# leonardsiegert/PULPo

Measured on AMD Instinct MI355X. Metric: volume-pairs/sec fwd+bwd, 160^3 fp32, higher is better.
Workload: dtype f32

## Files before the change

pulpo_amd/csrc/warp.hip:

```cpp
#include "common.h"
#include "sampling.h"

namespace {

using pulpo::Corner;
using pulpo::sample_coord;

template <int C>
__global__ __launch_bounds__(256) void warp_fwd_kernel(const float* __restrict__ df, const float* __restrict__ img, const float* __restrict__ add,
                                                         float* __restrict__ out, int B, int Dg, int Hg, int Wg, int Di, int Hi, int Wi, int Cr) {
    const long Vg = (long)Dg * Hg * Wg, Vi = (long)Di * Hi * Wi;
    const long total = (long)B * Vg;
    const int nch = C > 0 ? C : Cr;
    for (long e = blockIdx.x * (long)blockDim.x + threadIdx.x; e < total; e += (long)gridDim.x * blockDim.x) {
        const long b = B == 1 ? 0 : e / Vg, v = e - b * Vg;
        const int vi = (int)v;
        const int x = vi % Wg, y = (vi / Wg) % Hg, z = vi / (Wg * Hg);
        const float* d = df + b * 3 * Vg + v;
        const Corner cz = sample_coord((float)z, d[0], Dg, Di);
        const Corner cy = sample_coord((float)y, d[Vg], Hg, Hi);
        const Corner cx = sample_coord((float)x, d[2 * Vg], Wg, Wi);
        const long o00 = ((long)cz.i0 * Hi + cy.i0) * Wi, o01 = ((long)cz.i0 * Hi + cy.i1) * Wi;
        const long o10 = ((long)cz.i1 * Hi + cy.i0) * Wi, o11 = ((long)cz.i1 * Hi + cy.i1) * Wi;
        const float wz0 = 1.f - cz.f, wy0 = 1.f - cy.f, wx0 = 1.f - cx.f;
        for (int c = 0; c < nch; ++c) {
            const float* s = img + (b * nch + c) * Vi;
            float val = wz0 * wy0 * wx0 * s[o00 + cx.i0] + wz0 * wy0 * cx.f * s[o00 + cx.i1] + wz0 * cy.f * wx0 * s[o01 + cx.i0] +
                        wz0 * cy.f * cx.f * s[o01 + cx.i1] + cz.f * wy0 * wx0 * s[o10 + cx.i0] + cz.f * wy0 * cx.f * s[o10 + cx.i1] +
                        cz.f * cy.f * wx0 * s[o11 + cx.i0] + cz.f * cy.f * cx.f * s[o11 + cx.i1];
            const long oi = (b * nch + c) * Vg + v;
            if (add != nullptr) val += add[oi];
            out[oi] = val;
        }
    }
}

template <bool GDF_ATOMIC>
__global__ __launch_bounds__(256) void warp_bwd_kernel(const float* __restrict__ df, const float* __restrict__ img, const float* __restrict__ gout,
                                                         float* __restrict__ gdf, float* __restrict__ gimg, int B, int Dg, int Hg, int Wg, int Di,
                                                         int Hi, int Wi, int nch) {
    const long Vg = (long)Dg * Hg * Wg, Vi = (long)Di * Hi * Wi;
    const long total = (long)B * Vg;
    for (long e = blockIdx.x * (long)blockDim.x + threadIdx.x; e < total; e += (long)gridDim.x * blockDim.x) {
        const long b = B == 1 ? 0 : e / Vg, v = e - b * Vg;
        const int vi = (int)v;
        const int x = vi % Wg, y = (vi / Wg) % Hg, z = vi / (Wg * Hg);
        const float* d = df + b * 3 * Vg + v;
        const Corner cz = sample_coord((float)z, d[0], Dg, Di);
        const Corner cy = sample_coord((float)y, d[Vg], Hg, Hi);
        const Corner cx = sample_coord((float)x, d[2 * Vg], Wg, Wi);
        const long o00 = ((long)cz.i0 * Hi + cy.i0) * Wi, o01 = ((long)cz.i0 * Hi + cy.i1) * Wi;
        const long o10 = ((long)cz.i1 * Hi + cy.i0) * Wi, o11 = ((long)cz.i1 * Hi + cy.i1) * Wi;
        const float wz0 = 1.f - cz.f, wy0 = 1.f - cy.f, wx0 = 1.f - cx.f;
        float gz = 0.f, gy = 0.f, gx = 0.f;
        for (int c = 0; c < nch; ++c) {
            const float g = gout[(b * nch + c) * Vg + v];
            const float* s = img + (b * nch + c) * Vi;
            const float s000 = s[o00 + cx.i0], s001 = s[o00 + cx.i1], s010 = s[o01 + cx.i0], s011 = s[o01 + cx.i1];
            const float s100 = s[o10 + cx.i0], s101 = s[o10 + cx.i1], s110 = s[o11 + cx.i0], s111 = s[o11 + cx.i1];
            gz += g * (wy0 * wx0 * (s100 - s000) + wy0 * cx.f * (s101 - s001) + cy.f * wx0 * (s110 - s010) + cy.f * cx.f * (s111 - s011));
            gy += g * (wz0 * wx0 * (s010 - s000) + wz0 * cx.f * (s011 - s001) + cz.f * wx0 * (s110 - s100) + cz.f * cx.f * (s111 - s101));
            gx += g * (wz0 * wy0 * (s001 - s000) + wz0 * cy.f * (s011 - s010) + cz.f * wy0 * (s101 - s100) + cz.f * cy.f * (s111 - s110));
            if (gimg != nullptr) {
                float* q = gimg + (b * nch + c) * Vi;
                atomicAdd(q + o00 + cx.i0, g * wz0 * wy0 * wx0);
                atomicAdd(q + o00 + cx.i1, g * wz0 * wy0 * cx.f);
                atomicAdd(q + o01 + cx.i0, g * wz0 * cy.f * wx0);
                atomicAdd(q + o01 + cx.i1, g * wz0 * cy.f * cx.f);
                atomicAdd(q + o10 + cx.i0, g * cz.f * wy0 * wx0);
                atomicAdd(q + o10 + cx.i1, g * cz.f * wy0 * cx.f);
                atomicAdd(q + o11 + cx.i0, g * cz.f * cy.f * wx0);
                atomicAdd(q + o11 + cx.i1, g * cz.f * cy.f * cx.f);
            }
        }
        if (gdf != nullptr) {
            float* q = gdf + b * 3 * Vg + v;
            if constexpr (GDF_ATOMIC) {
                atomicAdd(q, gz * cz.dscale);
                atomicAdd(q + Vg, gy * cy.dscale);
                atomicAdd(q + 2 * Vg, gx * cx.dscale);
            } else {
                q[0] = gz * cz.dscale;
                q[Vg] = gy * cy.dscale;
                q[2 * Vg] = gx * cx.dscale;
            }
        }
    }
}

template <int R>
__global__ __launch_bounds__(256) void vecint_bwd_tile_kernel(const float* __restrict__ cur, const float* __restrict__ gout, float* __restrict__ gp,
                                                                int B, int D, int H, int W, int ntz, int nty, int ntx) {
    constexpr int TZ_ = 4, TY_ = 8, TX_ = 8;
    constexpr int BZ = TZ_ + 2 * R, BY = TY_ + 2 * R, BX = TX_ + 2 * R, BV = BZ * BY * BX;
    __shared__ float box[3 * BV];
    const int tid = threadIdx.x;
    int t = blockIdx.x;
    const int tx_ = t % ntx; t /= ntx;
    const int ty_ = t % nty; t /= nty;
    const int tz_ = t % ntz;
    const int b = t / ntz;
    const int z0 = tz_ * TZ_, y0 = ty_ * TY_, x0 = tx_ * TX_;
    const long V = (long)D * H * W;
    for (int j = tid; j < 3 * BV; j += 256) box[j] = 0.f;
    __syncthreads();
    const int z = z0 + (tid >> 6), y = y0 + ((tid >> 3) & 7), x = x0 + (tid & 7);
    const bool valid = z < D && y < H && x < W;
    const long v = valid ? ((long)z * H + y) * W + x : 0;
    const float* d = cur + (long)b * 3 * V + v;
    const Corner cz = sample_coord((float)z, valid ? d[0] : 0.f, D, D);
    const Corner cy = sample_coord((float)y, valid ? d[V] : 0.f, H, H);
    const Corner cx = sample_coord((float)x, valid ? d[2 * V] : 0.f, W, W);
    const float wz0 = 1.f - cz.f, wy0 = 1.f - cy.f, wx0 = 1.f - cx.f;
    const long o00 = ((long)cz.i0 * H + cy.i0) * W, o01 = ((long)cz.i0 * H + cy.i1) * W;
    const long o10 = ((long)cz.i1 * H + cy.i0) * W, o11 = ((long)cz.i1 * H + cy.i1) * W;
    const int lz0 = cz.i0 - z0 + R, lz1 = cz.i1 - z0 + R, ly0 = cy.i0 - y0 + R, ly1 = cy.i1 - y0 + R, lx0 = cx.i0 - x0 + R, lx1 = cx.i1 - x0 + R;
    const bool inbox = valid && lz0 >= 0 && lz1 < BZ && ly0 >= 0 && ly1 < BY && lx0 >= 0 && lx1 < BX;
    const int key = inbox ? (((lz0 * 32 + lz1) * 32 + ly0) * 32 + ly1) : -1;
    const int key_l = __shfl_up(key, 1, 64), lx1_l = __shfl_up(lx1, 1, 64);
    const bool take = inbox && (tid & 7) != 0 && key_l == key && lx1_l == lx0;
    const int take_r = __shfl_down((int)take, 1, 64);
    const bool give = (tid & 7) != 7 && take_r != 0;
    const int row = (tid >> 3) & 7;
    const int ky0 = inbox ? ((lz0 * 32 + lz1) * 32 + lx0) : -1, ky1 = (inbox && !give) ? ((lz0 * 32 + lz1) * 32 + lx1) : -1;
    const int ky0_u = __shfl_up(ky0, 8, 64), ky1_u = __shfl_up(ky1, 8, 64), ly1_u = __shfl_up(ly1, 8, 64);
    const bool take_y0 = row != 0 && ky0 >= 0 && ky0_u == ky0 && ly1_u == ly0;
    const bool take_y1 = row != 0 && ky1 >= 0 && ky1_u == ky1 && ly1_u == ly0;
    const int ty0_d = __shfl_down((int)take_y0, 8, 64), ty1_d = __shfl_down((int)take_y1, 8, 64);
    const bool give_y0 = row != 7 && ty0_d != 0, give_y1 = row != 7 && ty1_d != 0;
    float gz = 0.f, gy = 0.f, gx = 0.f;
    float gid[3];
#pragma unroll
    for (int c = 0; c < 3; ++c) {
        const float g = valid ? gout[((long)b * 3 + c) * V + v] : 0.f;
        gid[c] = g;
        if (valid) {
            const float* s = cur + ((long)b * 3 + c) * V;
            const float s000 = s[o00 + cx.i0], s001 = s[o00 + cx.i1], s010 = s[o01 + cx.i0], s011 = s[o01 + cx.i1];
            const float s100 = s[o10 + cx.i0], s101 = s[o10 + cx.i1], s110 = s[o11 + cx.i0], s111 = s[o11 + cx.i1];
            gz += g * (wy0 * wx0 * (s100 - s000) + wy0 * cx.f * (s101 - s001) + cy.f * wx0 * (s110 - s010) + cy.f * cx.f * (s111 - s011));
            gy += g * (wz0 * wx0 * (s010 - s000) + wz0 * cx.f * (s011 - s001) + cz.f * wx0 * (s110 - s100) + cz.f * cx.f * (s111 - s101));
            gx += g * (wz0 * wy0 * (s001 - s000) + wz0 * cy.f * (s011 - s010) + cz.f * wy0 * (s101 - s100) + cz.f * cy.f * (s111 - s110));
        }
        float a000 = g * wz0 * wy0 * wx0, a010 = g * wz0 * cy.f * wx0, a100 = g * cz.f * wy0 * wx0, a110 = g * cz.f * cy.f * wx0;
        const float a001 = g * wz0 * wy0 * cx.f, a011 = g * wz0 * cy.f * cx.f, a101 = g * cz.f * wy0 * cx.f, a111 = g * cz.f * cy.f * cx.f;
        const float t00 = __shfl_up(a001, 1, 64), t01 = __shfl_up(a011, 1, 64), t10 = __shfl_up(a101, 1, 64), t11 = __shfl_up(a111, 1, 64);
        if (take) { a000 += t00; a010 += t01; a100 += t10; a110 += t11; }
        float b001 = a001, b101 = a101;
        const float u010 = __shfl_up(a010, 8, 64), u110 = __shfl_up(a110, 8, 64), u011 = __shfl_up(a011, 8, 64), u111 = __shfl_up(a111, 8, 64);
        if (take_y0) { a000 += u010; a100 += u110; }
        if (take_y1) { b001 += u011; b101 += u111; }
        if (inbox) {
            float* q = box + c * BV;
            const int p00 = (lz0 * BY + ly0) * BX, p01 = (lz0 * BY + ly1) * BX, p10 = (lz1 * BY + ly0) * BX, p11 = (lz1 * BY + ly1) * BX;
            atomicAdd(q + p00 + lx0, a000);
            atomicAdd(q + p10 + lx0, a100);
            if (!give_y0) {
                atomicAdd(q + p01 + lx0, a010);
                atomicAdd(q + p11 + lx0, a110);
            }
            if (!give) {
                atomicAdd(q + p00 + lx1, b001);
                atomicAdd(q + p10 + lx1, b101);
                if (!give_y1) {
                    atomicAdd(q + p01 + lx1, a011);
                    atomicAdd(q + p11 + lx1, a111);
                }
            }
        } else if (valid) {
            float* q = gp + ((long)b * 3 + c) * V;
            atomicAdd(q + o00 + cx.i0, a000);
            atomicAdd(q + o00 + cx.i1, a001);
            atomicAdd(q + o01 + cx.i0, a010);
            atomicAdd(q + o01 + cx.i1, a011);
            atomicAdd(q + o10 + cx.i0, a100);
            atomicAdd(q + o10 + cx.i1, a101);
            atomicAdd(q + o11 + cx.i0, a110);
            atomicAdd(q + o11 + cx.i1, a111);
        }
    }
    if (valid) {
        const int own = ((z - z0 + R) * BY + (y - y0 + R)) * BX + (x - x0 + R);
        atomicAdd(box + own, gid[0] + gz * cz.dscale);
        atomicAdd(box + BV + own, gid[1] + gy * cy.dscale);
        atomicAdd(box + 2 * BV + own, gid[2] + gx * cx.dscale);
    }
    __syncthreads();
    for (int j = tid; j < 3 * BV; j += 256) {
        const float val = box[j];
        if (val == 0.f) continue;
        const int c = j / BV, r = j - c * BV;
        const int gz_ = z0 - R + r / (BY * BX), gy_ = y0 - R + (r / BX) % BY, gx_ = x0 - R + r % BX;
        if (gz_ >= 0 && gz_ < D && gy_ >= 0 && gy_ < H && gx_ >= 0 && gx_ < W)
            atomicAdd(gp + ((long)b * 3 + c) * V + ((long)gz_ * H + gy_) * W + gx_, val);
    }
}

__global__ __launch_bounds__(256) void scale_kernel(const float* __restrict__ in, float* __restrict__ out, float s, long n) {
    for (long e = blockIdx.x * (long)blockDim.x + threadIdx.x; e < n; e += (long)gridDim.x * blockDim.x) out[e] = in[e] * s;
}

constexpr int VI_THREADS = 1024, VI_MAXV = 8 * VI_THREADS;
__global__ __launch_bounds__(VI_THREADS) void vecint_fwd_lds_kernel(const float* __restrict__ v, float* __restrict__ work, int B, int D, int H, int W,
                                                                      int nsteps, float scale) {
    extern __shared__ float fld[];
    const int V = D * H * W, tid = threadIdx.x;
    const long b = blockIdx.x, n = (long)B * 3 * V;
    for (int i = tid; i < 3 * V; i += VI_THREADS) {
        const float val = v[b * 3 * V + i] * scale;
        fld[i] = val;
        work[b * 3 * V + i] = val;
    }
    __syncthreads();
    for (int k = 0; k < nsteps; ++k) {
        float nv[8][3];
#pragma unroll
        for (int j = 0; j < 8; ++j) {
            const int vox = tid + j * VI_THREADS;
            if (vox < V) pulpo::vecint_step_voxel(fld, V, vox, D, H, W, nv[j]);
        }
        __syncthreads();
        float* out = work + (long)(k + 1) * n + b * 3 * V;
#pragma unroll
        for (int j = 0; j < 8; ++j) {
            const int vox = tid + j * VI_THREADS;
            if (vox < V) {
#pragma unroll
                for (int c = 0; c < 3; ++c) {
                    fld[c * V + vox] = nv[j][c];
                    out[c * V + vox] = nv[j][c];
                }
            }
        }
        __syncthreads();
    }
}

inline int eblocks(long items) { return (int)std::max<long>(1, std::min<long>((items + 255) / 256, 8192)); }

__device__ __forceinline__ double fx_unit(const unsigned* maxbits) {
    const float m = __uint_as_float(*maxbits);
    if (!(m > 0.f) || !(m < INFINITY)) return 1.0;
    int ex;
    frexpf(m, &ex);
    return ldexp(1.0, 46 - ex);
}
__device__ __forceinline__ void fx_add(long long* p, float v, double unit) {
    atomicAdd(reinterpret_cast<unsigned long long*>(p), (unsigned long long)__double2ll_rn((double)v * unit));
}

__device__ __forceinline__ void block_absmax_to(float m, unsigned* out) {
    __shared__ float wm[4];
#pragma unroll
    for (int o = 32; o > 0; o >>= 1) m = fmaxf(m, __shfl_xor(m, o, 64));
    if ((threadIdx.x & 63) == 0) wm[threadIdx.x >> 6] = m;
    __syncthreads();
    if (threadIdx.x == 0) {
        const float t = fmaxf(fmaxf(wm[0], wm[1]), fmaxf(wm[2], wm[3]));
        if (t > 0.f) atomicMax(out, __float_as_uint(t));
    }
}
inline int fx_blocks(long items) { return (int)std::max<long>(1, std::min<long>((items + 255) / 256, 1024)); }

__global__ __launch_bounds__(256) void absmax_kernel(const float* __restrict__ g, long n, unsigned* __restrict__ out) {
    float m = 0.f;
    for (long e = blockIdx.x * (long)blockDim.x + threadIdx.x; e < n; e += (long)gridDim.x * blockDim.x) m = fmaxf(m, fabsf(g[e]));
    block_absmax_to(m, out);
}

template <bool SELF>
__global__ __launch_bounds__(256) void warp_bwd_fx_kernel(const float* __restrict__ df, const float* __restrict__ img, const float* __restrict__ gout,
                                                            float* __restrict__ gdf, long long* __restrict__ acc, const unsigned* __restrict__ maxbits,
                                                            int B, int Dg, int Hg, int Wg, int Di, int Hi, int Wi, int nch) {
    const long Vg = (long)Dg * Hg * Wg, Vi = (long)Di * Hi * Wi;
    const long total = (long)B * Vg;
    const double unit = fx_unit(maxbits);
    for (long e = blockIdx.x * (long)blockDim.x + threadIdx.x; e < total; e += (long)gridDim.x * blockDim.x) {
        const long b = B == 1 ? 0 : e / Vg, v = e - b * Vg;
        const int vi = (int)v;
        const int x = vi % Wg, y = (vi / Wg) % Hg, z = vi / (Wg * Hg);
        const float* d = df + b * 3 * Vg + v;
        const Corner cz = sample_coord((float)z, d[0], Dg, Di);
        const Corner cy = sample_coord((float)y, d[Vg], Hg, Hi);
        const Corner cx = sample_coord((float)x, d[2 * Vg], Wg, Wi);
        const long o00 = ((long)cz.i0 * Hi + cy.i0) * Wi, o01 = ((long)cz.i0 * Hi + cy.i1) * Wi;
        const long o10 = ((long)cz.i1 * Hi + cy.i0) * Wi, o11 = ((long)cz.i1 * Hi + cy.i1) * Wi;
        const float wz0 = 1.f - cz.f, wy0 = 1.f - cy.f, wx0 = 1.f - cx.f;
        float gz = 0.f, gy = 0.f, gx = 0.f;
        float gid[3] = {0.f, 0.f, 0.f};
        for (int c = 0; c < nch; ++c) {
            const float g = gout[(b * nch + c) * Vg + v];
            if (SELF && c < 3) gid[c] = g;
            const float* s = img + (b * nch + c) * Vi;
            const float s000 = s[o00 + cx.i0], s001 = s[o00 + cx.i1], s010 = s[o01 + cx.i0], s011 = s[o01 + cx.i1];
            const float s100 = s[o10 + cx.i0], s101 = s[o10 + cx.i1], s110 = s[o11 + cx.i0], s111 = s[o11 + cx.i1];
            gz += g * (wy0 * wx0 * (s100 - s000) + wy0 * cx.f * (s101 - s001) + cy.f * wx0 * (s110 - s010) + cy.f * cx.f * (s111 - s011));
            gy += g * (wz0 * wx0 * (s010 - s000) + wz0 * cx.f * (s011 - s001) + cz.f * wx0 * (s110 - s100) + cz.f * cx.f * (s111 - s101));
            gx += g * (wz0 * wy0 * (s001 - s000) + wz0 * cy.f * (s011 - s010) + cz.f * wy0 * (s101 - s100) + cz.f * cy.f * (s111 - s110));
            if (acc != nullptr) {
                long long* q = acc + (b * nch + c) * Vi;
                fx_add(q + o00 + cx.i0, g * wz0 * wy0 * wx0, unit);
                fx_add(q + o00 + cx.i1, g * wz0 * wy0 * cx.f, unit);
                fx_add(q + o01 + cx.i0, g * wz0 * cy.f * wx0, unit);
                fx_add(q + o01 + cx.i1, g * wz0 * cy.f * cx.f, unit);
                fx_add(q + o10 + cx.i0, g * cz.f * wy0 * wx0, unit);
                fx_add(q + o10 + cx.i1, g * cz.f * wy0 * cx.f, unit);
                fx_add(q + o11 + cx.i0, g * cz.f * cy.f * wx0, unit);
                fx_add(q + o11 + cx.i1, g * cz.f * cy.f * cx.f, unit);
            }
        }
        if (SELF) {
            long long* q = acc + b * 3 * Vg + v;
            fx_add(q, gid[0] + gz * cz.dscale, unit);
            fx_add(q + Vg, gid[1] + gy * cy.dscale, unit);
            fx_add(q + 2 * Vg, gid[2] + gx * cx.dscale, unit);
        } else if (gdf != nullptr) {
            float* q = gdf + b * 3 * Vg + v;
            q[0] = gz * cz.dscale;
            q[Vg] = gy * cy.dscale;
            q[2 * Vg] = gx * cx.dscale;
        }
    }
}

__global__ __launch_bounds__(256) void fx_to_float_kernel(long long* __restrict__ acc, float* __restrict__ out, long n, const unsigned* __restrict__ maxbits,
                                                            float post, unsigned* __restrict__ next_max) {
    const double inv = 1.0 / fx_unit(maxbits);
    float m = 0.f;
    for (long e = blockIdx.x * (long)blockDim.x + threadIdx.x; e < n; e += (long)gridDim.x * blockDim.x) {
        const float val = (float)((double)acc[e] * inv) * post;
        acc[e] = 0;
        out[e] = val;
        m = fmaxf(m, fabsf(val));
    }
    if (next_max != nullptr) block_absmax_to(m, next_max);
}

}

PULPO_API int pulpo_warp3d_fwd(const float* df, const float* img, float* out, int B, int C, int Dg, int Hg, int Wg, int Di, int Hi, int Wi,
                               void* stream) {
    PULPO_REQUIRE(df && img && out && B > 0 && C > 0, "warp3d_fwd: bad arguments");
    PULPO_REQUIRE(Dg >= 1 && Hg > 1 && Wg > 1 && Di > 0 && Hi > 0 && Wi > 0 && (Dg > 1 || Di == 1), "warp3d_fwd: grid H, W must be > 1 (depth 1 = 2-D form, with a depth-1 image)");
    PULPO_REQUIRE((long)Dg * Hg * Wg < (1L << 31), "warp3d_fwd: grids of 2^31 voxels and more are not supported");
    const long total = (long)B * Dg * Hg * Wg;
    hipStream_t st = (hipStream_t)stream;
    if (C == 1) hipLaunchKernelGGL(warp_fwd_kernel<1>, dim3(eblocks(total)), dim3(256), 0, st, df, img, nullptr, out, B, Dg, Hg, Wg, Di, Hi, Wi, C);
    else if (C == 3) hipLaunchKernelGGL(warp_fwd_kernel<3>, dim3(eblocks(total)), dim3(256), 0, st, df, img, nullptr, out, B, Dg, Hg, Wg, Di, Hi, Wi, C);
    else hipLaunchKernelGGL(warp_fwd_kernel<0>, dim3(eblocks(total)), dim3(256), 0, st, df, img, nullptr, out, B, Dg, Hg, Wg, Di, Hi, Wi, C);
    return pulpo::check_launch("warp3d_fwd");
}

PULPO_API int pulpo_warp3d_bwd(const float* df, const float* img, const float* gout, float* gdf, float* gimg, int B, int C, int Dg, int Hg, int Wg,
                               int Di, int Hi, int Wi, void* stream) {
    PULPO_REQUIRE(df && img && gout && B > 0 && C > 0, "warp3d_bwd: bad arguments");
    PULPO_REQUIRE(Dg >= 1 && Hg > 1 && Wg > 1 && (long)Dg * Hg * Wg < (1L << 31), "warp3d_bwd: grid H, W must be > 1 (and fewer than 2^31 voxels)");
    hipStream_t st = (hipStream_t)stream;
    if (gimg != nullptr) {
        hipError_t e = hipMemsetAsync(gimg, 0, sizeof(float) * (size_t)B * C * Di * Hi * Wi, st);
        if (e != hipSuccess) return pulpo::fail((int)e, "warp3d_bwd memset: %s", hipGetErrorString(e));
    }
    const long total = (long)B * Dg * Hg * Wg;
    hipLaunchKernelGGL(warp_bwd_kernel<false>, dim3(eblocks(total)), dim3(256), 0, st, df, img, gout, gdf, gimg, B, Dg, Hg, Wg, Di, Hi, Wi, C);
    return pulpo::check_launch("warp3d_bwd");
}

PULPO_API int pulpo_vecint_fwd(const float* v, float* work, int B, int D, int H, int W, int nsteps, void* stream) {
    PULPO_REQUIRE(v && work && B > 0 && D >= 1 && H > 1 && W > 1 && nsteps >= 0 && (long)D * H * W < (1L << 31), "vecint_fwd: bad arguments");
    hipStream_t st = (hipStream_t)stream;
    const long n = (long)B * 3 * D * H * W, total = (long)B * D * H * W;
    constexpr long VECINT_LDS_MAXV = 2048;
    static_assert(VECINT_LDS_MAXV <= VI_MAXV, "the one-launch form holds the whole field in LDS");
    if (total / B <= VECINT_LDS_MAXV && nsteps > 0) {
        const size_t lds = sizeof(float) * 3 * (size_t)(total / B);
        static bool attr_set = false;
        if (!attr_set) {
            hipError_t e = hipFuncSetAttribute(reinterpret_cast<const void*>(&vecint_fwd_lds_kernel), hipFuncAttributeMaxDynamicSharedMemorySize,
                                               (int)(sizeof(float) * 3 * VI_MAXV));
            if (e != hipSuccess) return pulpo::fail((int)e, "hipFuncSetAttribute(vecint_fwd_lds): %s", hipGetErrorString(e));
            attr_set = true;
        }
        hipLaunchKernelGGL(vecint_fwd_lds_kernel, dim3(B), dim3(VI_THREADS), lds, st, v, work, B, D, H, W, nsteps, 1.0f / (float)(1 << nsteps));
        return pulpo::check_launch("vecint_fwd_lds");
    }
    hipLaunchKernelGGL(scale_kernel, dim3(eblocks(n)), dim3(256), 0, st, v, work, 1.0f / (float)(1 << nsteps), n);
    int rc = pulpo::check_launch("vecint scale");
    if (rc) return rc;
    for (int k = 0; k < nsteps; ++k) {
        const float* cur = work + (long)k * n;
        hipLaunchKernelGGL(warp_fwd_kernel<3>, dim3(eblocks(total)), dim3(256), 0, st, cur, cur, cur, work + (long)(k + 1) * n, B, D, H, W, D, H, W, 3);
        rc = pulpo::check_launch("vecint step");
        if (rc) return rc;
    }
    return 0;
}

static bool vecint_bwd_tiled(int D, int H, int W) {
    constexpr int TILED_MIN = 8;
    return D >= TILED_MIN && H >= TILED_MIN && W >= TILED_MIN;
}

PULPO_API size_t pulpo_vecint_bwd_tmp_floats(int B, int D, int H, int W, int nsteps) {
    if (B <= 0 || D < 1 || H < 1 || W < 1 || nsteps <= 0) return 0;
    const size_t n = (size_t)B * 3 * D * H * W;
    return vecint_bwd_tiled(D, H, W) ? (size_t)nsteps * n : 2 * n;
}

PULPO_API int pulpo_vecint_bwd(const float* work, const float* gout, float* gin, float* tmp, int B, int D, int H, int W, int nsteps, void* stream) {
    PULPO_REQUIRE(work && gout && gin && B > 0 && D >= 1 && H > 1 && W > 1 && nsteps >= 0 && (long)D * H * W < (1L << 31), "vecint_bwd: bad arguments");
    PULPO_REQUIRE(tmp || pulpo_vecint_bwd_tmp_floats(B, D, H, W, nsteps) == 0, "vecint_bwd: scratch of pulpo_vecint_bwd_tmp_floats() floats required");
    hipStream_t st = (hipStream_t)stream;
    const long n = (long)B * 3 * D * H * W, total = (long)B * D * H * W;
    const float scale = 1.0f / (float)(1 << nsteps);
    const bool tiled = vecint_bwd_tiled(D, H, W);
    if (tiled && nsteps > 0) {
        hipError_t e = hipMemsetAsync(tmp, 0, sizeof(float) * n * nsteps, st);
        if (e != hipSuccess) return pulpo::fail((int)e, "vecint_bwd fill: %s", hipGetErrorString(e));
    }
    const float* g = gout;
    for (int k = nsteps - 1; k >= 0; --k) {
        const float* cur = work + (long)k * n;
        float* gp;
        if (tiled) {
            gp = tmp + (long)k * n;
            const int ntz = pulpo::cdiv(D, 4), nty = pulpo::cdiv(H, 8), ntx = pulpo::cdiv(W, 8);
            if (k == nsteps - 1 && (long)D * H * W >= 64L * 64 * 64)
                hipLaunchKernelGGL(vecint_bwd_tile_kernel<2>, dim3((unsigned)((long)B * ntz * nty * ntx)), dim3(256), 0, st, cur, g, gp, B, D, H, W, ntz, nty, ntx);
            else
                hipLaunchKernelGGL(vecint_bwd_tile_kernel<1>, dim3((unsigned)((long)B * ntz * nty * ntx)), dim3(256), 0, st, cur, g, gp, B, D, H, W, ntz, nty, ntx);
        } else {
            gp = tmp + (long)(k & 1) * n;
            hipError_t e = hipMemcpyAsync(gp, g, sizeof(float) * n, hipMemcpyDeviceToDevice, st);
            if (e != hipSuccess) return pulpo::fail((int)e, "vecint_bwd copy: %s", hipGetErrorString(e));
            hipLaunchKernelGGL(warp_bwd_kernel<true>, dim3(eblocks(total)), dim3(256), 0, st, cur, cur, g, gp, gp, B, D, H, W, D, H, W, 3);
        }
        int rc = pulpo::check_launch("vecint_bwd step");
        if (rc) return rc;
        g = gp;
    }
    hipLaunchKernelGGL(scale_kernel, dim3(eblocks(n)), dim3(256), 0, st, g, gin, scale, n);
    return pulpo::check_launch("vecint_bwd scale");
}

PULPO_API size_t pulpo_warp3d_bwd_det_ws_bytes(int B, int C, int Di, int Hi, int Wi) {
    if (B <= 0 || C <= 0 || Di < 1 || Hi < 1 || Wi < 1) return 0;
    return 256 + sizeof(long long) * (size_t)B * C * Di * Hi * Wi;
}

PULPO_API int pulpo_warp3d_bwd_det(const float* df, const float* img, const float* gout, float* gdf, float* gimg, void* ws, int B, int C, int Dg, int Hg,
                                   int Wg, int Di, int Hi, int Wi, void* stream) {
    PULPO_REQUIRE(df && img && gout && B > 0 && C > 0, "warp3d_bwd_det: bad arguments");
    PULPO_REQUIRE(Dg >= 1 && Hg > 1 && Wg > 1 && (long)Dg * Hg * Wg < (1L << 31), "warp3d_bwd_det: grid H, W must be > 1 (and fewer than 2^31 voxels)");
    PULPO_REQUIRE(ws != nullptr || gimg == nullptr, "warp3d_bwd_det: workspace of pulpo_warp3d_bwd_det_ws_bytes() bytes required for the image gradient");
    hipStream_t st = (hipStream_t)stream;
    const long total = (long)B * Dg * Hg * Wg, ni = (long)B * C * Di * Hi * Wi;
    if (gimg == nullptr) {
        hipLaunchKernelGGL(warp_bwd_kernel<false>, dim3(eblocks(total)), dim3(256), 0, st, df, img, gout, gdf, (float*)nullptr, B, Dg, Hg, Wg, Di, Hi, Wi, C);
        return pulpo::check_launch("warp3d_bwd_det");
    }
    unsigned* slots = (unsigned*)ws;
    long long* acc = (long long*)((char*)ws + 256);
    hipError_t e = hipMemsetAsync(ws, 0, 256 + sizeof(long long) * (size_t)ni, st);
    if (e != hipSuccess) return pulpo::fail((int)e, "warp3d_bwd_det memset: %s", hipGetErrorString(e));
    hipLaunchKernelGGL(absmax_kernel, dim3(fx_blocks((long)B * C * Dg * Hg * Wg)), dim3(256), 0, st, gout, (long)B * C * Dg * Hg * Wg, slots);
    hipLaunchKernelGGL(warp_bwd_fx_kernel<false>, dim3(eblocks(total)), dim3(256), 0, st, df, img, gout, gdf, acc, slots, B, Dg, Hg, Wg, Di, Hi, Wi, C);
    hipLaunchKernelGGL(fx_to_float_kernel, dim3(fx_blocks(ni)), dim3(256), 0, st, acc, gimg, ni, slots, 1.0f, (unsigned*)nullptr);
    return pulpo::check_launch("warp3d_bwd_det");
}

PULPO_API size_t pulpo_vecint_bwd_det_ws_bytes(int B, int D, int H, int W, int nsteps) {
    if (B <= 0 || D < 1 || H < 1 || W < 1 || nsteps <= 0) return 0;
    const size_t n = (size_t)B * 3 * D * H * W;
    return 256 + sizeof(long long) * n + 2 * sizeof(float) * n;
}

PULPO_API int pulpo_vecint_bwd_det(const float* work, const float* gout, float* gin, void* ws, int B, int D, int H, int W, int nsteps, void* stream) {
    PULPO_REQUIRE(work && gout && gin && B > 0 && D >= 1 && H > 1 && W > 1 && nsteps >= 0 && nsteps < 60 && (long)D * H * W < (1L << 31), "vecint_bwd_det: bad arguments");
    PULPO_REQUIRE(ws || nsteps == 0, "vecint_bwd_det: workspace of pulpo_vecint_bwd_det_ws_bytes() bytes required");
    hipStream_t st = (hipStream_t)stream;
    const long n = (long)B * 3 * D * H * W, total = (long)B * D * H * W;
    const float scale = 1.0f / (float)(1 << nsteps);
    if (nsteps == 0) {
        hipLaunchKernelGGL(scale_kernel, dim3(eblocks(n)), dim3(256), 0, st, gout, gin, scale, n);
        return pulpo::check_launch("vecint_bwd_det scale");
    }
    unsigned* slots = (unsigned*)ws;
    long long* acc = (long long*)((char*)ws + 256);
    float* buf[2] = {(float*)(acc + n), (float*)(acc + n) + n};
    hipError_t e = hipMemsetAsync(ws, 0, 256 + sizeof(long long) * (size_t)n, st);
    if (e != hipSuccess) return pulpo::fail((int)e, "vecint_bwd_det memset: %s", hipGetErrorString(e));
    hipLaunchKernelGGL(absmax_kernel, dim3(fx_blocks(n)), dim3(256), 0, st, gout, n, slots + (nsteps - 1));
    const float* g = gout;
    for (int k = nsteps - 1; k >= 0; --k) {
        const float* cur = work + (long)k * n;
        hipLaunchKernelGGL(warp_bwd_fx_kernel<true>, dim3(eblocks(total)), dim3(256), 0, st, cur, cur, g, (float*)nullptr, acc, slots + k, B, D, H, W, D, H, W, 3);
        float* out = k == 0 ? gin : buf[k & 1];
        hipLaunchKernelGGL(fx_to_float_kernel, dim3(fx_blocks(n)), dim3(256), 0, st, acc, out, n, slots + k, k == 0 ? scale : 1.0f, k == 0 ? (unsigned*)nullptr : slots + (k - 1));
        g = out;
    }
    return pulpo::check_launch("vecint_bwd_det");
}
```

Before: 39.58.

## Replace scatter-atomic vecint backward with halo-gather kernel and fold final scaling

The tiled vector-integration backward no longer scatters bilinear weights into a shared-memory box with LDS atomics followed by a global atomic flush. Each block instead stages per-voxel sample records (fractions, corner-membership bits, upstream gradient, field values) for the tile plus its halo in LDS. Each voxel then gathers contributions from its (2R+1)^3 neighbourhood, and only far-displaced voxels still scatter with global atomics. The final step writes straight into gin with the 1/2^n scale folded in, which removes the separate scale kernel, and one zero kernel replaces the memset. The cost is more LDS per block, a neighbourhood loop per voxel, and reading the halo's displacements and gradients redundantly.

```diff
diff --git a/pulpo_amd/csrc/warp.hip b/pulpo_amd/csrc/warp.hip
--- a/pulpo_amd/csrc/warp.hip
+++ b/pulpo_amd/csrc/warp.hip
@@ -89,11 +89,30 @@
 }
 
 template <int R>
-__global__ __launch_bounds__(256) void vecint_bwd_tile_kernel(const float* __restrict__ cur, const float* __restrict__ gout, float* __restrict__ gp,
-                                                                int B, int D, int H, int W, int ntz, int nty, int ntx) {
+__device__ __forceinline__ unsigned corner_bits(const Corner& c, int p) {
+    constexpr int NW = 2 * R + 1;
+    const int o0 = c.i0 - p + R, o1 = c.i1 - p + R;
+    return (o0 >= 0 && o1 < NW) ? (1u << o0) | (1u << (NW + o1)) : 0u;
+}
+
+template <int R>
+__device__ __forceinline__ float cell_weight(unsigned bits, float f, int axis, int d) {
+    constexpr int NW = 2 * R + 1;
+    const int p0 = axis * 2 * NW + R - d;
+    return (((bits >> p0) & 1u) ? 1.f - f : 0.f) + (((bits >> (p0 + NW)) & 1u) ? f : 0.f);
+}
+
+template <int R>
+__global__ __launch_bounds__(256) void vecint_bwd_gather_kernel(const float* __restrict__ cur, const float* __restrict__ gout, float* __restrict__ gp,
+                                                                  float oscale, int B, int D, int H, int W, int ntz, int nty, int ntx) {
     constexpr int TZ_ = 4, TY_ = 8, TX_ = 8;
-    constexpr int BZ = TZ_ + 2 * R, BY = TY_ + 2 * R, BX = TX_ + 2 * R, BV = BZ * BY * BX;
-    __shared__ float box[3 * BV];
+    constexpr int BZ = TZ_ + 2 * R, BY = TY_ + 2 * R, BX = TX_ + 2 * R, BV = BZ * BY * BX, NW = 2 * R + 1;
+    constexpr unsigned NEAR = 1u << 31;
+    static_assert(6 * NW < 32, "corner bits and the near bit share one word");
+    __shared__ float4 rec_w[BV];
+    __shared__ float4 rec_g[BV];
+    __shared__ float fld[3 * BV];
+    static_assert(sizeof(float) * 11 * BV <= 64 * 1024, "the records stay under 64 KB of LDS");
     const int tid = threadIdx.x;
     int t = blockIdx.x;
     const int tx_ = t % ntx; t /= ntx;
@@ -102,97 +121,111 @@
     const int b = t / ntz;
     const int z0 = tz_ * TZ_, y0 = ty_ * TY_, x0 = tx_ * TX_;
     const long V = (long)D * H * W;
-    for (int j = tid; j < 3 * BV; j += 256) box[j] = 0.f;
+    const float* curb = cur + (long)b * 3 * V;
+    const float* goutb = gout + (long)b * 3 * V;
+    float* gpb = gp + (long)b * 3 * V;
+
+    auto stage = [&](int j, int lz, int ly, int lx, Corner& cz, Corner& cy, Corner& cx, float g[3]) -> unsigned {
+        const int z = z0 - R + lz, y = y0 - R + ly, x = x0 - R + lx;
+        unsigned bits = 0u;
+        float d0 = 0.f, d1 = 0.f, d2 = 0.f;
+        cz = cy = cx = Corner{0, 0, 0.f, 0.f};
+        g[0] = g[1] = g[2] = 0.f;
+        if (z >= 0 && z < D && y >= 0 && y < H && x >= 0 && x < W) {
+            const long v = ((long)z * H + y) * W + x;
+            d0 = curb[v]; d1 = curb[V + v]; d2 = curb[2 * V + v];
+            g[0] = goutb[v]; g[1] = goutb[V + v]; g[2] = goutb[2 * V + v];
+            cz = sample_coord((float)z, d0, D, D);
+            cy = sample_coord((float)y, d1, H, H);
+            cx = sample_coord((float)x, d2, W, W);
+            const unsigned bz = corner_bits<R>(cz, z), by = corner_bits<R>(cy, y), bx = corner_bits<R>(cx, x);
+            if (bz != 0u && by != 0u && bx != 0u) bits = NEAR | bz | (by << (2 * NW)) | (bx << (4 * NW));
+        }
+        rec_w[j] = make_float4(cz.f, cy.f, cx.f, __uint_as_float(bits));
+        rec_g[j] = make_float4(g[0], g[1], g[2], 0.f);
+        fld[j] = d0; fld[BV + j] = d1; fld[2 * BV + j] = d2;
+        return bits;
+    };
+
+    const int hz = tid >> 6, hy = (tid >> 3) & 7, hx = tid & 7;
+    const int z = z0 + hz, y = y0 + hy, x = x0 + hx;
+    const bool valid = z < D && y < H && x < W;
+    const int own = ((hz + R) * BY + (hy + R)) * BX + (hx + R);
+    Corner cz, cy, cx;
+    float gid[3];
+    const unsigned hbits = stage(own, hz + R, hy + R, hx + R, cz, cy, cx, gid);
+    for (int j = tid; j < BV; j += 256) {
+        const int lz = j / (BY * BX), r = j - lz * (BY * BX), ly = r / BX, lx = r - ly * BX;
+        if ((unsigned)(lz - R) < (unsigned)TZ_ && (unsigned)(ly - R) < (unsigned)TY_ && (unsigned)(lx - R) < (unsigned)TX_) continue;
+        Corner rz, ry, rx;
+        float rg[3];
+        stage(j, lz, ly, lx, rz, ry, rx, rg);
+    }
     __syncthreads();
-    const int z = z0 + (tid >> 6), y = y0 + ((tid >> 3) & 7), x = x0 + (tid & 7);
-    const bool valid = z < D && y < H && x < W;
-    const long v = valid ? ((long)z * H + y) * W + x : 0;
-    const float* d = cur + (long)b * 3 * V + v;
-    const Corner cz = sample_coord((float)z, valid ? d[0] : 0.f, D, D);
-    const Corner cy = sample_coord((float)y, valid ? d[V] : 0.f, H, H);
-    const Corner cx = sample_coord((float)x, valid ? d[2 * V] : 0.f, W, W);
+
+    constexpr int UY = R == 1 ? NW : 1;
+    float acc[3] = {0.f, 0.f, 0.f};
+#pragma unroll 1
+    for (int dz = -R; dz <= R; ++dz)
+#pragma unroll UY
+        for (int dy = -R; dy <= R; ++dy)
+#pragma unroll
+            for (int dx = -R; dx <= R; ++dx) {
+                const int j = own + (dz * BY + dy) * BX + dx;
+                const float4 w = rec_w[j];
+                const float4 g = rec_g[j];
+                const unsigned bits = __float_as_uint(w.w);
+                const float wt = cell_weight<R>(bits, w.x, 0, dz) * cell_weight<R>(bits, w.y, 1, dy) * cell_weight<R>(bits, w.z, 2, dx);
+                acc[0] += g.x * wt;
+                acc[1] += g.y * wt;
+                acc[2] += g.z * wt;
+            }
+    if (!valid) return;
+
+    const long v = ((long)z * H + y) * W + x;
     const float wz0 = 1.f - cz.f, wy0 = 1.f - cy.f, wx0 = 1.f - cx.f;
-    const long o00 = ((long)cz.i0 * H + cy.i0) * W, o01 = ((long)cz.i0 * H + cy.i1) * W;
-    const long o10 = ((long)cz.i1 * H + cy.i0) * W, o11 = ((long)cz.i1 * H + cy.i1) * W;
-    const int lz0 = cz.i0 - z0 + R, lz1 = cz.i1 - z0 + R, ly0 = cy.i0 - y0 + R, ly1 = cy.i1 - y0 + R, lx0 = cx.i0 - x0 + R, lx1 = cx.i1 - x0 + R;
-    const bool inbox = valid && lz0 >= 0 && lz1 < BZ && ly0 >= 0 && ly1 < BY && lx0 >= 0 && lx1 < BX;
-    const int key = inbox ? (((lz0 * 32 + lz1) * 32 + ly0) * 32 + ly1) : -1;
-    const int key_l = __shfl_up(key, 1, 64), lx1_l = __shfl_up(lx1, 1, 64);
-    const bool take = inbox && (tid & 7) != 0 && key_l == key && lx1_l == lx0;
-    const int take_r = __shfl_down((int)take, 1, 64);
-    const bool give = (tid & 7) != 7 && take_r != 0;
-    const int row = (tid >> 3) & 7;
-    const int ky0 = inbox ? ((lz0 * 32 + lz1) * 32 + lx0) : -1, ky1 = (inbox && !give) ? ((lz0 * 32 + lz1) * 32 + lx1) : -1;
-    const int ky0_u = __shfl_up(ky0, 8, 64), ky1_u = __shfl_up(ky1, 8, 64), ly1_u = __shfl_up(ly1, 8, 64);
-    const bool take_y0 = row != 0 && ky0 >= 0 && ky0_u == ky0 && ly1_u == ly0;
-    const bool take_y1 = row != 0 && ky1 >= 0 && ky1_u == ky1 && ly1_u == ly0;
-    const int ty0_d = __shfl_down((int)take_y0, 8, 64), ty1_d = __shfl_down((int)take_y1, 8, 64);
-    const bool give_y0 = row != 7 && ty0_d != 0, give_y1 = row != 7 && ty1_d != 0;
+    const bool is_near = (hbits & NEAR) != 0u;
+    const long o00 = is_near ? own + ((cz.i0 - z) * BY + (cy.i0 - y)) * BX - x : ((long)cz.i0 * H + cy.i0) * W;
+    const long o01 = is_near ? own + ((cz.i0 - z) * BY + (cy.i1 - y)) * BX - x : ((long)cz.i0 * H + cy.i1) * W;
+    const long o10 = is_near ? own + ((cz.i1 - z) * BY + (cy.i0 - y)) * BX - x : ((long)cz.i1 * H + cy.i0) * W;
+    const long o11 = is_near ? own + ((cz.i1 - z) * BY + (cy.i1 - y)) * BX - x : ((long)cz.i1 * H + cy.i1) * W;
     float gz = 0.f, gy = 0.f, gx = 0.f;
-    float gid[3];
 #pragma unroll
     for (int c = 0; c < 3; ++c) {
-        const float g = valid ? gout[((long)b * 3 + c) * V + v] : 0.f;
-        gid[c] = g;
-        if (valid) {
-            const float* s = cur + ((long)b * 3 + c) * V;
-            const float s000 = s[o00 + cx.i0], s001 = s[o00 + cx.i1], s010 = s[o01 + cx.i0], s011 = s[o01 + cx.i1];
-            const float s100 = s[o10 + cx.i0], s101 = s[o10 + cx.i1], s110 = s[o11 + cx.i0], s111 = s[o11 + cx.i1];
-            gz += g * (wy0 * wx0 * (s100 - s000) + wy0 * cx.f * (s101 - s001) + cy.f * wx0 * (s110 - s010) + cy.f * cx.f * (s111 - s011));
-            gy += g * (wz0 * wx0 * (s010 - s000) + wz0 * cx.f * (s011 - s001) + cz.f * wx0 * (s110 - s100) + cz.f * cx.f * (s111 - s101));
-            gx += g * (wz0 * wy0 * (s001 - s000) + wz0 * cy.f * (s011 - s010) + cz.f * wy0 * (s101 - s100) + cz.f * cy.f * (s111 - s110));
-        }
-        float a000 = g * wz0 * wy0 * wx0, a010 = g * wz0 * cy.f * wx0, a100 = g * cz.f * wy0 * wx0, a110 = g * cz.f * cy.f * wx0;
-        const float a001 = g * wz0 * wy0 * cx.f, a011 = g * wz0 * cy.f * cx.f, a101 = g * cz.f * wy0 * cx.f, a111 = g * cz.f * cy.f * cx.f;
-        const float t00 = __shfl_up(a001, 1, 64), t01 = __shfl_up(a011, 1, 64), t10 = __shfl_up(a101, 1, 64), t11 = __shfl_up(a111, 1, 64);
-        if (take) { a000 += t00; a010 += t01; a100 += t10; a110 += t11; }
-        float b001 = a001, b101 = a101;
-        const float u010 = __shfl_up(a010, 8, 64), u110 = __shfl_up(a110, 8, 64), u011 = __shfl_up(a011, 8, 64), u111 = __shfl_up(a111, 8, 64);
-        if (take_y0) { a000 += u010; a100 += u110; }
-        if (take_y1) { b001 += u011; b101 += u111; }
-        if (inbox) {
-            float* q = box + c * BV;
-            const int p00 = (lz0 * BY + ly0) * BX, p01 = (lz0 * BY + ly1) * BX, p10 = (lz1 * BY + ly0) * BX, p11 = (lz1 * BY + ly1) * BX;
-            atomicAdd(q + p00 + lx0, a000);
-            atomicAdd(q + p10 + lx0, a100);
-            if (!give_y0) {
-                atomicAdd(q + p01 + lx0, a010);
-                atomicAdd(q + p11 + lx0, a110);
-            }
-            if (!give) {
-                atomicAdd(q + p00 + lx1, b001);
-                atomicAdd(q + p10 + lx1, b101);
-                if (!give_y1) {
-                    atomicAdd(q + p01 + lx1, a011);
-                    atomicAdd(q + p11 + lx1, a111);
-                }
-            }
-        } else if (valid) {
-            float* q = gp + ((long)b * 3 + c) * V;
-            atomicAdd(q + o00 + cx.i0, a000);
-            atomicAdd(q + o00 + cx.i1, a001);
-            atomicAdd(q + o01 + cx.i0, a010);
-            atomicAdd(q + o01 + cx.i1, a011);
-            atomicAdd(q + o10 + cx.i0, a100);
-            atomicAdd(q + o10 + cx.i1, a101);
-            atomicAdd(q + o11 + cx.i0, a110);
-            atomicAdd(q + o11 + cx.i1, a111);
-        }
-    }
-    if (valid) {
-        const int own = ((z - z0 + R) * BY + (y - y0 + R)) * BX + (x - x0 + R);
-        atomicAdd(box + own, gid[0] + gz * cz.dscale);
-        atomicAdd(box + BV + own, gid[1] + gy * cy.dscale);
-        atomicAdd(box + 2 * BV + own, gid[2] + gx * cx.dscale);
-    }
-    __syncthreads();
-    for (int j = tid; j < 3 * BV; j += 256) {
-        const float val = box[j];
-        if (val == 0.f) continue;
-        const int c = j / BV, r = j - c * BV;
-        const int gz_ = z0 - R + r / (BY * BX), gy_ = y0 - R + (r / BX) % BY, gx_ = x0 - R + r % BX;
-        if (gz_ >= 0 && gz_ < D && gy_ >= 0 && gy_ < H && gx_ >= 0 && gx_ < W)
-            atomicAdd(gp + ((long)b * 3 + c) * V + ((long)gz_ * H + gy_) * W + gx_, val);
+        const float g = gid[c];
+        float s000, s001, s010, s011, s100, s101, s110, s111;
+        if (is_near) {
+            const float* s = fld + c * BV;
+            s000 = s[o00 + cx.i0]; s001 = s[o00 + cx.i1]; s010 = s[o01 + cx.i0]; s011 = s[o01 + cx.i1];
+            s100 = s[o10 + cx.i0]; s101 = s[o10 + cx.i1]; s110 = s[o11 + cx.i0]; s111 = s[o11 + cx.i1];
+        } else {
+            const float* s = curb + c * V;
+            s000 = s[o00 + cx.i0]; s001 = s[o00 + cx.i1]; s010 = s[o01 + cx.i0]; s011 = s[o01 + cx.i1];
+            s100 = s[o10 + cx.i0]; s101 = s[o10 + cx.i1]; s110 = s[o11 + cx.i0]; s111 = s[o11 + cx.i1];
+            float* q = gpb + c * V;
+            const float go = g * oscale;
+            atomicAdd(q + o00 + cx.i0, go * wz0 * wy0 * wx0);
+            atomicAdd(q + o00 + cx.i1, go * wz0 * wy0 * cx.f);
+            atomicAdd(q + o01 + cx.i0, go * wz0 * cy.f * wx0);
+            atomicAdd(q + o01 + cx.i1, go * wz0 * cy.f * cx.f);
+            atomicAdd(q + o10 + cx.i0, go * cz.f * wy0 * wx0);
+            atomicAdd(q + o10 + cx.i1, go * cz.f * wy0 * cx.f);
+            atomicAdd(q + o11 + cx.i0, go * cz.f * cy.f * wx0);
+            atomicAdd(q + o11 + cx.i1, go * cz.f * cy.f * cx.f);
+        }
+        gz += g * (wy0 * wx0 * (s100 - s000) + wy0 * cx.f * (s101 - s001) + cy.f * wx0 * (s110 - s010) + cy.f * cx.f * (s111 - s011));
+        gy += g * (wz0 * wx0 * (s010 - s000) + wz0 * cx.f * (s011 - s001) + cz.f * wx0 * (s110 - s100) + cz.f * cx.f * (s111 - s101));
+        gx += g * (wz0 * wy0 * (s001 - s000) + wz0 * cy.f * (s011 - s010) + cz.f * wy0 * (s101 - s100) + cz.f * cy.f * (s111 - s110));
+    }
+    atomicAdd(gpb + v, (acc[0] + gid[0] + gz * cz.dscale) * oscale);
+    atomicAdd(gpb + V + v, (acc[1] + gid[1] + gy * cy.dscale) * oscale);
+    atomicAdd(gpb + 2 * V + v, (acc[2] + gid[2] + gx * cx.dscale) * oscale);
+}
+
+__global__ __launch_bounds__(256) void zero2_kernel(float* __restrict__ a, long na, float* __restrict__ b, long nb) {
+    for (long e = blockIdx.x * (long)blockDim.x + threadIdx.x; e < na + nb; e += (long)gridDim.x * blockDim.x) {
+        if (e < na) a[e] = 0.f;
+        else b[e - na] = 0.f;
     }
 }
 
@@ -412,28 +445,35 @@
     hipStream_t st = (hipStream_t)stream;
     const long n = (long)B * 3 * D * H * W, total = (long)B * D * H * W;
     const float scale = 1.0f / (float)(1 << nsteps);
-    const bool tiled = vecint_bwd_tiled(D, H, W);
-    if (tiled && nsteps > 0) {
-        hipError_t e = hipMemsetAsync(tmp, 0, sizeof(float) * n * nsteps, st);
-        if (e != hipSuccess) return pulpo::fail((int)e, "vecint_bwd fill: %s", hipGetErrorString(e));
+    if (vecint_bwd_tiled(D, H, W) && nsteps > 0) {
+        const long nz = (long)(nsteps - 1) * n;
+        hipLaunchKernelGGL(zero2_kernel, dim3(eblocks(nz + n)), dim3(256), 0, st, tmp + n, nz, gin, n);
+        int rc = pulpo::check_launch("vecint_bwd fill");
+        if (rc) return rc;
+        const int ntz = pulpo::cdiv(D, 4), nty = pulpo::cdiv(H, 8), ntx = pulpo::cdiv(W, 8);
+        const dim3 grid((unsigned)((long)B * ntz * nty * ntx));
+        const float* g = gout;
+        for (int k = nsteps - 1; k >= 0; --k) {
+            const float* cur = work + (long)k * n;
+            float* gp = k == 0 ? gin : tmp + (long)k * n;
+            const float os = k == 0 ? scale : 1.0f;
+            if (k == nsteps - 1 && (long)D * H * W >= 64L * 64 * 64)
+                hipLaunchKernelGGL(vecint_bwd_gather_kernel<2>, grid, dim3(256), 0, st, cur, g, gp, os, B, D, H, W, ntz, nty, ntx);
+            else
+                hipLaunchKernelGGL(vecint_bwd_gather_kernel<1>, grid, dim3(256), 0, st, cur, g, gp, os, B, D, H, W, ntz, nty, ntx);
+            rc = pulpo::check_launch("vecint_bwd step");
+            if (rc) return rc;
+            g = gp;
+        }
+        return 0;
     }
     const float* g = gout;
     for (int k = nsteps - 1; k >= 0; --k) {
         const float* cur = work + (long)k * n;
-        float* gp;
-        if (tiled) {
-            gp = tmp + (long)k * n;
-            const int ntz = pulpo::cdiv(D, 4), nty = pulpo::cdiv(H, 8), ntx = pulpo::cdiv(W, 8);
-            if (k == nsteps - 1 && (long)D * H * W >= 64L * 64 * 64)
-                hipLaunchKernelGGL(vecint_bwd_tile_kernel<2>, dim3((unsigned)((long)B * ntz * nty * ntx)), dim3(256), 0, st, cur, g, gp, B, D, H, W, ntz, nty, ntx);
-            else
-                hipLaunchKernelGGL(vecint_bwd_tile_kernel<1>, dim3((unsigned)((long)B * ntz * nty * ntx)), dim3(256), 0, st, cur, g, gp, B, D, H, W, ntz, nty, ntx);
-        } else {
-            gp = tmp + (long)(k & 1) * n;
-            hipError_t e = hipMemcpyAsync(gp, g, sizeof(float) * n, hipMemcpyDeviceToDevice, st);
-            if (e != hipSuccess) return pulpo::fail((int)e, "vecint_bwd copy: %s", hipGetErrorString(e));
-            hipLaunchKernelGGL(warp_bwd_kernel<true>, dim3(eblocks(total)), dim3(256), 0, st, cur, cur, g, gp, gp, B, D, H, W, D, H, W, 3);
-        }
+        float* gp = tmp + (long)(k & 1) * n;
+        hipError_t e = hipMemcpyAsync(gp, g, sizeof(float) * n, hipMemcpyDeviceToDevice, st);
+        if (e != hipSuccess) return pulpo::fail((int)e, "vecint_bwd copy: %s", hipGetErrorString(e));
+        hipLaunchKernelGGL(warp_bwd_kernel<true>, dim3(eblocks(total)), dim3(256), 0, st, cur, cur, g, gp, gp, B, D, H, W, D, H, W, 3);
         int rc = pulpo::check_launch("vecint_bwd step");
         if (rc) return rc;
         g = gp;
```

Measured after the change: 39.70 (median of 6 runs). Within noise of the previous version (+0.3%).
